# ansys/pychemkin

Hardware: AMD Instinct MI355X
Metric: reactor integrations/sec (GRI-3.0 const-P ignition) (higher is better)
Workload: dtype f64; 1 GPU; configs[2]: GRI-3.0 CONP CH4/air ignition sweep 64 T0 x 32 phi x 32 P per GPU; reactors_per_gpu=65536, ignition=TIFP, parallelism=shard-by-condition x1

## Files before the change

pychemkin_amd/csrc/ckmi_reactor.hpp:

```cpp
#pragma once
#include "ckmi_device.hpp"
#include "ckmi_image.hpp"
#include "../../include/ckmi.h"

namespace ckmi {

constexpr int QMAX = 5;
constexpr double ETAMX1 = 10000.0, ETAMX2 = 10.0, ETAMX3 = 10.0, ETAMXF = 0.2, ETAMIN = 0.1, ETACF = 0.25;
constexpr double ADDON = 1e-6, BIAS1 = 6.0, BIAS2 = 6.0, BIAS3 = 10.0, ONEPSM = 1.000001;
constexpr int SMALL_NST = 10, MXNCF = 10, MXNEF = 7, MXNEF1 = 3, SMALL_NEF = 2, LONG_WAIT = 10, MAXCOR = 3;
constexpr double CRDOWN = 0.3, DGMAX = 0.3, RDIV = 2.0, THRESH = 1.5, CORTES = 0.1;
constexpr int MSBP = 20, MSBJ = 15;
constexpr double UROUND = 2.220446049250313e-16, NNEG_TOL = 0.01;

constexpr int VL = WAVE;
struct WaveLds {
  int base;
  __device__ __forceinline__ double* C() const { return lds_at<double>(base); }
  __device__ __forceinline__ double* gRT() const { return lds_at<double>(base + 8 * VL); }
  __device__ __forceinline__ double* hRT() const { return lds_at<double>(base + 16 * VL); }
  __device__ __forceinline__ double* wdot() const { return lds_at<double>(base + 24 * VL); }
  __device__ __forceinline__ double* dwdT() const { return lds_at<double>(base + 32 * VL); }
  __device__ __forceinline__ double* ek() const { return lds_at<double>(base + 40 * VL); }
  __device__ __forceinline__ double* Mg() const { return lds_at<double>(base + 48 * VL); }
// ... 713 lines not shown
    if (wave_lane() >= n) b = 0.0;
    const double bp = bpermute(permv, b);
    double s0 = 0.0, s1 = 0.0;
#pragma unroll
    for (int j = 0; j < N; j += 2) {
      s0 = fma((double)a[j], bcast(bp, j), s0);
      if (j + 1 < N) s1 = fma((double)a[j + 1], bcast(bp, j + 1), s1);
    }
    return bpermute(permv, s0 + s1);
  }
};

template <int S>
__device__ __forceinline__ double pick(const double (&v)[S], int i) {
  double r = v[0];
#pragma unroll
  for (int k = 1; k < S; ++k) r = (i == k) ? v[k] : r;
  return r;
}

__device__ __forceinline__ double eta_root(double x, int p) {
  return (double)exp2f(log2f((float)x) / (float)p);
}

struct BdfS {
  double h, hscale, hprime, eta, etamax, hmax_inv, hmin, tn, rl1, gamma, gammap, gamrat, crate, acnrm, saved_tq5, hu;
  double l[QMAX + 1], tq[6], tau[QMAX + 2];
  int q, qprime, qwait, L, nst, nstlp, nstlj, jcur, ncf_tot, nef_tot, nlu, nfe, nje, nni;
  double rtol, atol;
  int nneg;
};

template <int ST>
struct ZnLdsT {
  int base;
  __device__ __forceinline__ double& operator[](int j) const { return *lds_at<double>(base + j * ST * 8); }
};
using ZnLds = ZnLdsT<WAVE>;
constexpr int ZN_BYTES = (QMAX + 1) * WAVE * 8;

template <int ST>
struct BdfT {
  ZnLdsT<ST> zn;
  double ewt, acor, tempv, ftemp, y;
};
using Bdf = BdfT<WAVE>;

__device__ __forceinline__ double wrms_lane(double v, double ewt, int n) {
  const double x = v * ewt;
  return sqrt(wave_sum(x * x) / n);
}

template <class BB, class SS>
__device__ __forceinline__ void bdf_rescale(BB& b, SS& S) {
  double factor = S.eta;
#pragma unroll
  for (int j = 1; j <= QMAX; ++j) {
    if (j <= S.q) {
      b.zn[j] *= factor;
      factor *= S.eta;
    }
  }
  S.h = S.hscale * S.eta;
  S.hscale = S.h;
}

template <class BB, class SS>
__device__ __forceinline__ void bdf_predict(BB& b, SS& S) {
  S.tn += S.h;
  const int q = S.q;
  double z[QMAX + 1];
#pragma unroll
  for (int j = 0; j <= QMAX; ++j) z[j] = b.zn[j];
#pragma unroll
  for (int k = 1; k <= QMAX; ++k)
#pragma unroll
    for (int j = QMAX; j >= 1; --j)
      if (j >= k) z[j - 1] = (k <= q && j <= q) ? z[j - 1] + z[j] : z[j - 1];
#pragma unroll
  for (int j = 0; j < QMAX; ++j) b.zn[j] = z[j];
}

template <class BB, class SS>
__device__ __forceinline__ void bdf_restore(BB& b, SS& S, double saved_t) {
  S.tn = saved_t;
  const int q = S.q;
  double z[QMAX + 1];
#pragma unroll
  for (int j = 0; j <= QMAX; ++j) z[j] = b.zn[j];
#pragma unroll
  for (int k = 1; k <= QMAX; ++k)
#pragma unroll
    for (int j = QMAX; j >= 1; --j)
      if (j >= k) z[j - 1] = (k <= q && j <= q) ? z[j - 1] - z[j] : z[j - 1];
#pragma unroll
  for (int j = 0; j < QMAX; ++j) b.zn[j] = z[j];
}

template <class BB, class SS>
__device__ __forceinline__ void bdf_set(BB& b, SS& S) {
  const int q = S.q;
  const double h = S.h;
  double tau[QMAX + 1];
#pragma unroll
  for (int i = 0; i <= QMAX; ++i) tau[i] = S.tau[i];
  double l[QMAX + 1];
  double xi_inv = 1.0, xistar_inv = 1.0, alpha0 = -1.0, alpha0_hat = -1.0, hsum = h;
  l[0] = l[1] = 1.0;
#pragma unroll
  for (int i = 2; i <= QMAX; ++i) l[i] = 0.0;
  if (q > 1) {
#pragma unroll
    for (int j = 2; j < QMAX; ++j) {
      if (j < q) {
        hsum += tau[j - 1];
        xi_inv = h / hsum;
// ... 6 lines not shown
    alpha0 -= 1.0 / q;
    xistar_inv = -l[1] - alpha0;
    double tq1 = tau[0];
#pragma unroll
    for (int i = 1; i <= QMAX; ++i) tq1 = (i == q - 1) ? tau[i] : tq1;
    hsum += tq1;
    xi_inv = h / hsum;
    alpha0_hat = -l[1] - xi_inv;
#pragma unroll
    for (int i = QMAX; i >= 1; --i)
      if (i <= q) l[i] += l[i - 1] * xistar_inv;
  }
  double lq = l[0];
#pragma unroll
  for (int i = 1; i <= QMAX; ++i) lq = (i == q) ? l[i] : lq;
#pragma unroll
  for (int i = 0; i <= QMAX; ++i) S.l[i] = l[i];
  const double A1 = 1.0 - alpha0_hat + alpha0;
  const double A2 = 1.0 + q * A1;
  const double tq2 = fabs(A1 / (alpha0 * A2));
  S.tq[2] = tq2;
  S.tq[5] = fabs(A2 * xistar_inv / (lq * xi_inv));
  if (S.qwait == 1) {
    if (q > 1) {
      const double Cc = xistar_inv / lq;
      const double A3 = alpha0 + 1.0 / q;
      const double A4 = alpha0_hat + xi_inv;
      const double Cpinv = (1.0 - A4 + A3) / A3;
      S.tq[1] = fabs(Cc * Cpinv);
    } else {
      S.tq[1] = 1.0;
    }
    double tq = tau[0];
#pragma unroll
    for (int i = 1; i <= QMAX; ++i) tq = (i == q) ? tau[i] : tq;
    hsum += tq;
    xi_inv = h / hsum;
    const double A5 = alpha0 - 1.0 / (q + 1);
    const double A6 = alpha0_hat - xi_inv;
    const double Cppinv = (1.0 - A6 + A5) / A2;
    S.tq[3] = fabs(Cppinv / (xi_inv * (q + 2) * A5));
  }
  S.tq[4] = CORTES / tq2;
  const double rl1 = 1.0 / l[1];
  const double gamma = h * rl1;
  S.rl1 = rl1;
  S.gamma = gamma;
  if (S.nst == 0) S.gammap = gamma;
  S.gamrat = (S.nst > 0) ? gamma / S.gammap : 1.0;
}


template <class BB, class SS>
__device__ __forceinline__ void bdf_adjust_order(BB& b, SS& S, int deltaq) {
  const int q = S.q;
#pragma unroll
  for (int i = 0; i <= QMAX; ++i) S.l[i] = 0.0;
  S.l[2] = 1.0;
  if (deltaq == 1) {
    double alpha1 = 1.0, prod = 1.0, xiold = 1.0, alpha0 = -1.0, hsum = S.hscale;
#pragma unroll
    for (int j = 1; j < QMAX; ++j) {
      if (j < q) {
        hsum += S.tau[j + 1];
        const double xi = hsum / S.hscale;
        prod *= xi;
        alpha0 -= 1.0 / (j + 1);
        alpha1 += 1.0 / xi;
#pragma unroll
        for (int i = QMAX; i >= 2; --i)
          if (i <= j + 2) S.l[i] = S.l[i] * xiold + S.l[i - 1];
        xiold = xi;
      }
    }
    const double A1 = (-alpha0 - alpha1) / prod;
    const double znL = A1 * b.zn[QMAX];
#pragma unroll
    for (int j = 2; j <= QMAX; ++j)
      if (j <= q) b.zn[j] += S.l[j] * znL;
#pragma unroll
    for (int j = 1; j <= QMAX; ++j)
      if (j == q + 1) b.zn[j] = znL;
  } else {
    double hsum = 0.0;
#pragma unroll
    for (int j = 1; j <= QMAX; ++j) {
      if (j <= q - 2) {
        hsum += S.tau[j];
        const double xi = hsum / S.hscale;
#pragma unroll
        for (int i = QMAX; i >= 2; --i)
          if (i <= j + 2) S.l[i] = S.l[i] * xi + S.l[i - 1];
      }
    }
    double znq = 0.0;
#pragma unroll
    for (int j = 0; j <= QMAX; ++j)
      if (j == q) znq = b.zn[j];
#pragma unroll
    for (int j = 2; j <= QMAX; ++j)
      if (j < q) b.zn[j] -= S.l[j] * znq;
  }
}

template <class BB, class SS>
__device__ __forceinline__ double dky0_lane(const BB& b, const SS& S, double t) {
  const double sc = (t - S.tn) / S.h;
  double v = 0.0;
#pragma unroll
  for (int j = QMAX; j >= 0; --j)
    if (j <= S.q) v = b.zn[j] + sc * v;
  return v;
}

}
```

pychemkin_amd/csrc/ckmi_reactor_kernel.hpp:

```cpp
#pragma once
#include <hip/hip_runtime.h>

#include <algorithm>
#include <string>
#include <type_traits>

#include "../../include/ckmi.h"
#include "ckmi_reactor.hpp"
#include "ckmi_run.hpp"
#include "ckmi_internal.hpp"

namespace {
using namespace ckmi;

enum { PH_RHS = 0, PH_JAC = 1, PH_LU = 2, PH_SOLVE = 3, PH_TOTAL = 4, PH_STATE = 8, PH_N = 48 };
#ifdef CKMI_PHASE_TIMERS
__device__ unsigned long long* g_phase_buf = nullptr;
#define PH_T0() const unsigned long long _ph0 = __builtin_amdgcn_s_memtime()
#define PH_ADD(slot) ph[slot] += __builtin_amdgcn_s_memtime() - _ph0
#else
#define PH_T0() (void)0
#define PH_ADD(slot) (void)0
#endif

// ... 55 lines not shown
  const ckmi_reactor_cfg* __restrict__ cfg = &dcfg->c;
  const int oJ = img.bytes;
  const int olock = oJ + jlock_offset(N);
  if (threadIdx.x == 0) *lds_at<int>(olock) = 0;
  stage_image(0, img);
  const MechView V = make_view(0, img);
  const int wid = threadIdx.x / WAVE;
  const int lane = threadIdx.x % WAVE;
  const int ows = oJ + jscratch_bytes<N>() + wid * (slice_bytes(img.G) + (PSR ? 8 * VL : 0));
  WaveLds L;
  L.base = ows;
  double* const Yin = PSR ? lds_at<double>(ows + slice_bytes(img.G)) : nullptr;
  const int oS = ows + slice_vec_bytes(img.G);
  BdfS& S = *lds_at<BdfS>(oS);
  Ctl& c = *lds_at<Ctl>(oS + align16((int)sizeof(BdfS)));
  Ign& g = *lds_at<Ign>(oS + align16((int)sizeof(BdfS)) + align16((int)sizeof(Ctl)));
  constexpr int RWAVES = rwaves(F64);
  float* Jg = reinterpret_cast<float*>(jws) + ((size_t)blockIdx.x * RWAVES + wid) * N * WAVE;
  const int KK = V.KK;
  const int n = KK + 1;
  const bool isp = lane >= 1 && lane <= KK;
  const bool act = lane < n;
  RunCtx& R = *lds_at<RunCtx>(oS + align16((int)sizeof(BdfS)) + align16((int)sizeof(Ctl)) + align16((int)sizeof(Ign)));
  R.cfg = cfg;
  std::conditional_t<F64, NewtonMatrixGJ64<N>, NewtonMatrixF32S<N>> M;
  Bdf b;
  b.zn.base = oS + align16((int)sizeof(BdfS)) + align16((int)sizeof(Ctl)) + align16((int)sizeof(Ign)) +
              align16((int)sizeof(RunCtx)) + lane * 8;
  double fe = 0.0, y_e = 0.0, t_e = 0.0;
  bool with_j = false;
#ifdef CKMI_PHASE_TIMERS
  unsigned long long ph[8] = {0, 0, 0, 0, 0, 0, 0, 0};
  unsigned long long t_r0 = 0;
  unsigned long long* phs = lds_at<unsigned long long>(oS + align16((int)sizeof(BdfS)) + align16((int)sizeof(Ctl)) +
                                                     align16((int)sizeof(Ign)) + align16((int)sizeof(RunCtx)) +
                                                     ZN_BYTES);
#endif
  int st = ST_NEXT;

#define REQUEST_F(T_, Y_, NEXT_) \
  do {                           \
    t_e = (T_);                  \
    y_e = (Y_);                  \
    with_j = false;              \
    st = (NEXT_);                \
    want = true;                 \
  } while (0)
#define START_BEGIN(T_, Y_, TOUT_, H0_)                                 \
  do {                                                                 \
    S.tn = (T_);                                                       \
    b.zn[0] = act ? (Y_) : 0.0;                                        \
    _Pragma("unroll") for (int j_ = 1; j_ <= QMAX; ++j_) b.zn[j_] = 0.0; \
    b.ewt = act ? 1.0 / (S.rtol * fabs(b.zn[0]) + S.atol) : 0.0;       \
    c.st_tout = (TOUT_);                                               \
    R.tsel = 0.5 * (S.tn + c.st_tout);                                 \
    c.st_h0 = (H0_);                                                   \
    REQUEST_F(S.tn, b.zn[0], ST_START_F);                              \
  } while (0)

  auto psr_resid = [&](double f, double y) -> double {
    if constexpr (PSR) {
      const double T = bcast(y, 0);
      const double sYW = wave_sum(isp ? y * V.rwt()[lane - 1] : 0.0);
      const double tau = R.pfr == 4 ? R.P0 / (RU * T * sYW * R.G) : 1.0 / R.G;
      const double den = lane == 0 ? io.ss_rtol * T : io.ss_rtol * fabs(y) + io.ss_atol;
      const double v = act ? tau * fabs(f) / den : 0.0;
      return __ballot(act && !(v == v)) != 0 ? __builtin_nan("") : wave_max(v);
    } else {
      return 0.0;
    }
  };

  for (;;) {
    bool want = false;
    while (!want && st != ST_EXIT) {
#ifdef CKMI_PHASE_TIMERS
      const int st_in = st;
      const unsigned long long t_st = __builtin_amdgcn_s_memtime();
#endif
      if constexpr (PSR) {
        if (st == ST_FINISH && c.stopped == 0) {
          c.stopped = 2;
          REQUEST_F(S.tn, b.zn[0], ST_PSR_END_F);
          continue;
        }
        if (st > ST_EXIT) {
          S.nfe++;
          const double res = psr_resid(fe, y_e);
          if (st == ST_PSR_END_F) {
            c.avar_last = res;
            if (c.status == 0 && !(res <= 1.0)) c.status = CKMI_RUN_NOT_STEADY;
            st = ST_FINISH;
            continue;
          }
          const bool polishing = st == ST_PSR_POLISH_F;
          if (res <= 1.0) {
            if (polishing) b.zn[0] = b.y;
            c.avar_last = res;
            c.stopped = 1;
            st = ST_FINISH;
            continue;
          }
          if (polishing ? (c.nadap < PSR_POLISH_ITERS && res < PSR_POLISH_RATE * c.delp) : res <= PSR_POLISH_MAX) {
            c.nadap = polishing ? c.nadap + 1 : 1;
            c.delp = res;
            const double d = M.solve(act ? S.gammap * fe : 0.0, n);
            S.nni++;
// ... 62 lines not shown
          R.mass = R.rho0 * R.V0;
          if (PF && R.pfr == 1) {
            R.G = R.rho0 * R.V0;
            R.Pm = R.P0 + R.G * R.V0;
          }
          if constexpr (PSR) {
            const bool vgiven = io.mode == 2;
            R.conp = 1;
            R.pfr = vgiven ? 4 : 3;
            const double Tin = io.Tin[r], mdot = io.mdot[r];
            const double yi = isp ? io.Yin[(size_t)r * KK + lane - 1] : 0.0;
            if (isp) Yin[lane - 1] = yi;
            const double hin = isp ? nasa7_img(V, lane - 1, Tin, log(Tin), 1.0 / Tin).hRT * RU * Tin * V.rwt()[lane - 1] : 0.0;
            R.Pm = wave_sum(yi * hin);
            R.G = vgiven ? mdot / R.V0 : 1.0 / R.V0;
            R.mass = vgiven ? R.rho0 * R.V0 : R.V0 * mdot;
            wave_lds_sync();
          }
          R.gfac = cfg->gfac;
          R.qloss = cfg->qloss;
          R.htc = cfg->htc;
          R.areaq = cfg->areaq;
          R.tamb = cfg->tamb;
          R.nq = cfg->prof2_kind == 1 ? cfg->nprof2 : 0;
          R.na = cfg->prof2_kind == 2 ? cfg->nprof2 : cfg->nprof3;
          R.a_t = cfg->prof2_kind == 2 ? cfg->prof2_t : cfg->prof3_t;
          R.a_v = cfg->prof2_kind == 2 ? cfg->prof2_v : cfg->prof3_v;
          {
            const int ar = io.afac_rxn ? io.afac_rxn[r] : -1;
            R.pslot = (ar >= 0 && ar < img.II) ? img.slot_of[ar] : -1;
            R.plnf = R.pslot >= 0 ? log(io.afac[r]) : 0.0;
          }
          c.nadap = 0;
          c.avar_last = bcast(yl, cfg->avar > 0 ? cfg->avar : 0);
          c.T0 = T0;
          c.yguard = dcfg->guard_y;
          c.tguard_lo = dcfg->guard_tlo;
          c.tguard_hi = dcfg->guard_thi;
          S.rtol = cfg->rtol;
          S.atol = cfg->atol;
          S.nneg = cfg->nneg;
          S.ncf_tot = S.nef_tot = S.nlu = S.nfe = S.nje = S.nni = 0;
          c.tend = cfg->t_end;
          if constexpr (PSR) {
            if (!(c.tend > 0.0)) c.tend = 1000.0 * (R.pfr == 4 ? R.rho0 / R.G : 1.0 / R.G);
          }
          c.hmax = cfg->hmax > 0.0 ? cfg->hmax : c.tend / 100.0;
          S.hmax_inv = 1.0 / c.hmax;
          S.hmin = 0.0;
          c.ncrit = n_crit(dcfg);
          c.icrit = 0;
          c.first = 1;
          c.max_steps = cfg->max_steps > 0 ? cfg->max_steps : 200000;
#ifdef CKMI_PHASE_TIMERS
#pragma unroll
          for (int k = 0; k < 8; ++k) ph[k] = 0;
          if (lane < 40) phs[lane] = 0;
          t_r0 = __builtin_amdgcn_s_memtime();
#endif
          START_BEGIN(0.0, yl, crit_time(dcfg, c.tend, 0), cfg->h0);
          break;
        }
        case ST_START_F: {
          b.zn[1] = act ? fe : 0.0;
          S.nfe++;
          if (c.st_h0 > 0.0) {
            c.st_h = c.st_h0;
            st = ST_START_FINISH;
            break;
          }
          const double t0 = S.tn, tout = c.st_tout;
          const double tdist = fabs(tout - t0);
          const double tround = UROUND * fmax(fabs(t0), fabs(tout));
          const double hlb = 100.0 * tround;
          double hub = 0.1 * tdist;
          const double num = act ? fabs(b.zn[1]) : 0.0;
          const double den = 0.1 * fabs(b.zn[0]) + S.atol;
          const double hub_inv = wave_max(act ? num / (den > 0 ? den : 1e-300) : 0.0);
          if (hub * hub_inv > 1.0) hub = 1.0 / hub_inv;
          const double hg = sqrt(hlb * hub);
          if (hub < hlb) {
            c.st_h = hg;
            st = ST_START_FINISH;
            break;
          }
          c.is_t0 = t0;
          c.is_hg = hg;
          c.is_hub = hub;
          c.is_hlb = hlb;
          c.is_count = 1;
          REQUEST_F(t0 + hg, b.zn[0] + hg * b.zn[1], ST_INITSTEP_F);
          break;
        }
        case ST_INITSTEP_F: {
          S.nfe++;
          const double hg = c.is_hg, hub = c.is_hub;
          const double f1 = act ? (fe - b.zn[1]) / hg : 0.0;
          const double yddnrm = wrms_lane(f1, b.ewt, n);
          double hnew = (yddnrm * hub * hub > 2.0) ? sqrt(2.0 / yddnrm) : sqrt(hg * hub);
          bool done = c.is_count == 4;
          if (!done) {
            const double hrat = hnew / hg;
            if (hrat > 0.5 && hrat < 2.0) {
              done = true;
            } else if (c.is_count >= 2 && hrat > 2.0) {
              hnew = hg;
// ... 17 lines not shown
          double h = c.st_h;
          if (h > c.hmax) h = c.hmax;
          if (h > c.st_tout - S.tn) h = c.st_tout - S.tn;
          b.zn[1] *= h;
          S.h = S.hscale = S.hprime = h;
          S.q = S.qprime = 1;
          S.L = 2;
          S.qwait = S.L;
          S.etamax = ETAMX1;
          S.nst = 0;
          S.nstlp = 0;
          S.nstlj = 0;
          S.jcur = 0;
          S.crate = 1.0;
          S.gammap = S.gamma = S.h;
          S.gamrat = 1.0;
          S.saved_tq5 = 0.0;
#pragma unroll
          for (int i = 0; i <= QMAX + 1; ++i) S.tau[i] = 0.0;
#pragma unroll
          for (int i = 0; i < 6; ++i) S.tq[i] = 0.0;
          S.hu = 0.0;
          st = ST_STEP_BEGIN;
          if (c.first) {
            c.first = 0;
            g.mode = cfg->ign_mode;
            g.comp = (g.mode == 4) ? 1 + cfg->ign_species : 0;
            g.found = g.started = g.have_prev = g.have_next = 0;
            g.thresh = 0.0;
            g.best = -1e300;
            g.tbest = g.tprev = g.vprev = g.tnext = g.vnext = g.tlast = g.vlast = 0.0;
            g.tau = -1.0;
            if (g.mode == 2) g.thresh = c.T0 + cfg->ign_val;
            if (g.mode == 3) g.thresh = cfg->ign_val;
            c.isave = 0;
            while (c.isave < io.nsave && io.t_save[c.isave] <= 0.0) {
              if (act) io.y_save[((size_t)c.r * io.nsave + c.isave) * n + lane] = b.zn[0];
              c.isave++;
            }
            c.status = 0;
            c.nst = 0;
            c.stopped = 0;
            if (g.mode == 1 || g.mode == 4) REQUEST_F(0.0, b.zn[0], ST_IGN0_F);
          }
          break;
        }
        case ST_IGN0_F: {
          S.nfe++;
          ign_peak_update(g, 0.0, g.mode == 1 ? bcast(fe, 0) : bcast(b.zn[0], g.comp));
          st = ST_STEP_BEGIN;
          break;
        }
        case ST_STEP_BEGIN: {
          if (!(S.tn < c.tend * (1.0 - 1e-15))) {
            st = ST_FINISH;
            break;
          }

          c.tc = crit_time(dcfg, c.tend, c.icrit);
          if (S.tn + S.hprime > c.tc) {
            const double hp = c.tc - S.tn;
            S.eta = hp / S.h;
            if (S.nst > 0) {
              S.hprime = hp;
            } else {
              bdf_rescale(b, S);
              S.hprime = S.h;
            }
          }
          b.ewt = act ? 1.0 / (S.rtol * fabs(b.zn[0]) + S.atol) : 0.0;
          c.told = S.tn;
          c.saved_t = S.tn;
          c.ncf = c.nef = 0;
          c.nflag = NF_FIRST;
          if (S.nst > 0 && S.hprime != S.h) {
            if (S.qprime != S.q) {
              bdf_adjust_order(b, S, S.qprime - S.q);
              S.q = S.qprime;
              S.L = S.q + 1;
              S.qwait = S.L;
            }
            bdf_rescale(b, S);
          }
          st = ST_STEP_ATTEMPT;
          break;
        }
        case ST_STEP_ATTEMPT: {
          bdf_predict(b, S);
          bdf_set(b, S);
          c.convfail = (c.nflag == NF_FIRST || c.nflag == NF_ERR_FAIL) ? CF_NONE : CF_OTHER;
          c.call_setup = (c.nflag != NF_FIRST) || S.nst == 0 || S.nst >= S.nstlp + MSBP || fabs(S.gamrat - 1.0) > DGMAX;
          st = ST_NLS_ATTEMPT;
          break;
        }
        case ST_NLS_ATTEMPT: {
          b.y = b.zn[0];
          if (c.call_setup) {
            const double dgamma = fabs(S.gamma / S.gammap - 1.0);
            const int jbad = S.nst == 0 || S.nst >= S.nstlj + MSBJ || (c.convfail == CF_BAD_J && dgamma < DGMAX) ||
                             c.convfail == CF_OTHER;
            if (jbad) {
              REQUEST_F(S.tn, b.y, ST_NLS_J);
              with_j = true;
              break;
            }
          }
          REQUEST_F(S.tn, b.y, ST_NLS_F);
          break;
        }
        case ST_NLS_F: {
          b.ftemp = fe;
          S.nfe++;
          if (!c.call_setup) {
            b.acor = 0.0;
            c.delp = 0.0;
            c.mm = 0;
            st = ST_NEWTON_ITER;
            break;
          }
          S.jcur = 0;
          st = ST_SETUP;
          break;
        }
        case ST_NLS_J: {
          b.ftemp = fe;
          {
            const double* Jsh = lds_at<const double>(oJ);
#pragma unroll 2
            for (int j = 0; j < N; ++j) Jg[j * WAVE + lane] = (float)Jsh[j * LDJ + lane];
          }
          wave_lds_sync();
          if (lane == 0) atomicExch(lds_at<int>(olock), 0);
          S.nfe += 2;
          S.nje++;
          S.nstlj = S.nst;
          S.jcur = 1;
          st = ST_SETUP;
          break;
        }
        case ST_SETUP: {
#ifdef CKMI_PHASE_TIMERS
          const unsigned long long t0 = __builtin_amdgcn_s_memtime();
#endif
          const bool ok = M.build_factor(Jg, WAVE, S.gamma, n, L.base + 32 * VL);
#ifdef CKMI_PHASE_TIMERS
          ph[PH_LU] += __builtin_amdgcn_s_memtime() - t0;
#endif
          S.nlu++;
          S.crate = 1.0;
          S.gammap = S.gamma;
          S.gamrat = 1.0;
          S.nstlp = S.nst;
          if (!ok) {
            st = ST_STEP_CONVFAIL;
            break;
          }
          b.acor = 0.0;
          c.delp = 0.0;
          c.mm = 0;
          st = ST_NEWTON_ITER;
          break;
        }
        case ST_NEWTON_ITER: {
          const double rhs = act ? S.gamma * b.ftemp - (S.rl1 * b.zn[1] + b.acor) : 0.0;
#ifdef CKMI_PHASE_TIMERS
          const unsigned long long t0 = __builtin_amdgcn_s_memtime();
#endif
          double x = M.solve(rhs, n);
#ifdef CKMI_PHASE_TIMERS
          ph[PH_SOLVE] += __builtin_amdgcn_s_memtime() - t0;
#endif
          S.nni++;
          if (S.gamrat != 1.0) x *= 2.0 / (1.0 + S.gamrat);
          if (!act) x = 0.0;
          const double z0 = b.zn[0];
          b.acor += x;
          b.y = z0 + b.acor;
          const bool neg = S.nneg && act && lane >= 1 && b.y < 0.0;
          double nv[4];
          {
            const double xe = x * b.ewt, ae = b.acor * b.ewt, ne = neg ? b.y * b.ewt : 0.0;
            const double fe2 = neg ? z0 * b.ewt : ae;
            nv[0] = xe * xe;
            nv[1] = ae * ae;
            nv[2] = ne * ne;
            nv[3] = fe2 * fe2;
          }
          wave_sum_multi<4>(nv, lane);
          const double del = sqrt(nv[0] / n);
          if (c.mm > 0) S.crate = fmax(CRDOWN * S.crate, del / c.delp);
          const double dcon = del * fmin(1.0, S.crate) / S.tq[4];
          if (dcon <= 1.0) {
            bool negfail = false, negfix = false;
            if (S.nneg && nv[2] > 0.0) {
              if (sqrt(nv[2] / n) > NNEG_TOL) {
                negfail = true;
              } else {
                negfix = true;
                if (neg) {
                  b.y = 0.0;
                  b.acor = -z0;
                }
              }
            }
            if (negfail) {
              c.failed = 2;
              st = ST_NLS_FAIL;
              break;
            }
            S.acnrm = (c.mm == 0 && !negfix) ? del : sqrt((negfix ? nv[3] : nv[1]) / n);
            S.jcur = 0;
            st = ST_ERRTEST;
            break;
          }
          c.mm++;
          if (c.mm == MAXCOR || (c.mm >= 2 && del > RDIV * c.delp)) {
            c.failed = 1;
            st = ST_NLS_FAIL;
            break;
          }
          c.delp = del;
          REQUEST_F(S.tn, b.y, ST_NEWTON_F);
          break;
        }
        case ST_NEWTON_F: {
          b.ftemp = fe;
          S.nfe++;
          st = ST_NEWTON_ITER;
          break;
        }
        case ST_NLS_FAIL: {
          if (c.failed == 1 && !S.jcur) {
            c.convfail = CF_BAD_J;
            c.call_setup = 1;
            st = ST_NLS_ATTEMPT;
          } else {
            st = ST_STEP_CONVFAIL;
          }
          break;
        }
        case ST_STEP_CONVFAIL: {
          c.ncf++;
          S.ncf_tot++;
          S.etamax = 1.0;
          bdf_restore(b, S, c.saved_t);
          if (fabs(S.h) <= S.hmin * ONEPSM || c.ncf == MXNCF) {
            c.rc = CKMI_RUN_CONVFAIL;
            st = ST_STEP_END;
            break;
          }
          S.eta = fmax(ETACF, S.hmin / fabs(S.h));
          c.nflag = NF_CONV_FAIL;
          bdf_rescale(b, S);
          st = ST_STEP_ATTEMPT;
          break;
        }
        case ST_ERRTEST: {
          c.dsm = S.acnrm * S.tq[2];
          if (c.dsm <= 1.0) {
            st = ST_STEP_COMPLETE;
            break;
          }
          c.nef++;
          S.nef_tot++;
          c.nflag = NF_ERR_FAIL;
          bdf_restore(b, S, c.saved_t);
          if (fabs(S.h) <= S.hmin * ONEPSM || c.nef == MXNEF) {
            c.rc = CKMI_RUN_ERRTEST;
            st = ST_STEP_END;
            break;
          }
          S.etamax = 1.0;
          st = ST_STEP_ATTEMPT;
          if (c.nef <= MXNEF1) {
            S.eta = 1.0 / (eta_root(BIAS2 * c.dsm, S.L) + ADDON);
            S.eta = fmax(ETAMIN, fmax(S.eta, S.hmin / fabs(S.h)));
            if (c.nef >= SMALL_NEF) S.eta = fmin(S.eta, ETAMXF);
            bdf_rescale(b, S);
            break;
          }
          if (S.q > 1) {
            S.eta = fmax(ETAMIN, S.hmin / fabs(S.h));
            bdf_adjust_order(b, S, -1);
            S.L = S.q;
            S.q--;
            S.qwait = S.L;
            bdf_rescale(b, S);
            break;
          }
          S.eta = fmax(ETAMIN, S.hmin / fabs(S.h));
          S.h *= S.eta;
          S.hscale = S.h;
          S.qwait = LONG_WAIT;
          REQUEST_F(S.tn, b.zn[0], ST_ERR_F);
          break;
        }
        case ST_ERR_F: {
          S.nfe++;
          b.zn[1] = act ? S.h * fe : 0.0;
          st = ST_STEP_ATTEMPT;
          break;
        }
        case ST_STEP_COMPLETE: {
          const double dsm = c.dsm;
          S.nst++;
          c.nst++;
          S.hu = S.h;
#pragma unroll
          for (int i = QMAX; i >= 2; --i)
            if (i <= S.q) S.tau[i] = S.tau[i - 1];
          if (S.q == 1 && S.nst > 1) S.tau[2] = S.tau[1];
          S.tau[1] = S.h;
          double ddn = 0.0, dup = 0.0;
          if (S.etamax != 1.0 && S.qwait == 1) {
            const bool qm = S.q > 1, qp = S.q != QMAX && S.saved_tq5 != 0.0;
            double cquot = 0.0;
            if (qp) {
              const double hr = S.h / S.tau[2];
              double hrL = hr;
              for (int j = 1; j < S.L; ++j) hrL *= hr;
              cquot = (S.tq[5] / S.saved_tq5) * hrL;
            }
            double ov[2];
            {
              double znq = 0.0, lq = 0.0;
#pragma unroll
              for (int j = 0; j <= QMAX; ++j)
                if (j == S.q) {
                  znq = b.zn[j];
                  lq = S.l[j];
                }
              const double a = (act && qm) ? (znq + lq * b.acor) * b.ewt : 0.0;
              const double t = (act && qp) ? (b.acor - cquot * b.zn[QMAX]) * b.ewt : 0.0;
              ov[0] = a * a;
              ov[1] = t * t;
            }
            wave_sum_multi<2>(ov, lane);
            ddn = sqrt(ov[0] / n) * S.tq[1];
            dup = sqrt(ov[1] / n) * S.tq[3];
          }
          if (dcfg->npe) elem_project_wave(V, dcfg->npe, c.eb0, S.rtol, b.zn[0], b.acor, lane, L.ek());
#pragma unroll
          for (int j = 0; j <= QMAX; ++j)
            if (j <= S.q) b.zn[j] += S.l[j] * b.acor;
          S.qwait--;
          if (S.qwait == 1 && S.q != QMAX) {
            b.zn[QMAX] = b.acor;
            S.saved_tq5 = S.tq[5];
          }
          if (S.etamax == 1.0) {
            if (S.qwait < 2) S.qwait = 2;
            S.qprime = S.q;
            S.hprime = S.h;
            S.eta = 1.0;
          } else {
            const double etaq = 1.0 / (eta_root(BIAS2 * dsm, S.L) + ADDON);
            if (S.qwait != 0) {
              S.eta = etaq;
              S.qprime = S.q;
            } else {
              S.qwait = 2;
              double etaqm1 = 0.0, etaqp1 = 0.0;
              if (S.q > 1) etaqm1 = 1.0 / (eta_root(BIAS1 * ddn, S.q) + ADDON);
              if (S.q != QMAX && S.saved_tq5 != 0.0) etaqp1 = 1.0 / (eta_root(BIAS3 * dup, S.L + 1) + ADDON);
              const double etam = fmax(etaqm1, fmax(etaq, etaqp1));
              if (etam < THRESH) {
                S.eta = 1.0;
                S.qprime = S.q;
              } else if (etam == etaq) {
                S.eta = etaq;
                S.qprime = S.q;
              } else if (etam == etaqm1) {
                S.eta = etaqm1;
                S.qprime = S.q - 1;
              } else {
                S.eta = etaqp1;
                S.qprime = S.q + 1;
                b.zn[QMAX] = b.acor;
              }
            }
            if (S.eta < THRESH) {
              S.eta = 1.0;
              S.hprime = S.h;
            } else {
              S.eta = fmin(S.eta, S.etamax);
              S.eta /= fmax(1.0, fabs(S.h) * S.hmax_inv * S.eta);
              S.hprime = S.h * S.eta;
            }
          }
          S.etamax = (S.nst <= SMALL_NST) ? ETAMX2 : ETAMX3;
          {
            const double z0 = b.zn[0];
            const bool bad = isp ? -z0 > c.yguard
                                 : (lane == 0 && R.energy == 1 && !(z0 >= c.tguard_lo && z0 <= c.tguard_hi));
            c.rc = __ballot(bad) != 0 ? CKMI_RUN_RUNAWAY : 0;
          }
          if constexpr (PF) {
            if (R.pfr == 1 && R.npv == 0 && c.rc == 0) {
              const double z0 = b.zn[0];
              const double sYW = wave_sum(isp ? z0 * V.rwt()[lane - 1] : 0.0);
              if (R.Pm * R.Pm - 4.0 * R.G * R.G * RU * bcast(z0, 0) * sYW < 0.0) c.rc = CKMI_RUN_CHOKED;
            }
          }
          st = ST_STEP_END;
          break;
        }
        case ST_STEP_END: {
          if (c.rc != 0) {
            c.status = c.rc;
            st = ST_FINISH;
            break;
          }
          const double tn = S.tn;
          while (c.isave < io.nsave && io.t_save[c.isave] <= tn) {
            const double ys = dky0_lane(b, S, io.t_save[c.isave]);
            if (act) io.y_save[((size_t)c.r * io.nsave + c.isave) * n + lane] = ys;
            c.isave++;
          }
          if (g.mode == 1) {
            ign_peak_update(g, tn, bcast(b.zn[1], 0) / S.h);
          } else if (g.mode == 4) {
            ign_peak_update(g, tn, bcast(b.zn[0], g.comp));
          } else if ((g.mode == 2 || g.mode == 3) && !g.found && bcast(b.zn[0], 0) >= g.thresh) {
            double lo = c.told, hi = tn;
            for (int it = 0; it < 60; ++it) {
              const double mid = 0.5 * (lo + hi);
              if (bcast(dky0_lane(b, S, mid), 0) >= g.thresh) hi = mid;
              else lo = mid;
            }
            g.found = 1;
            g.tau = hi;
          }
          st = ST_STEP_BEGIN;
          if (cfg->ign_stop) {
            if ((g.mode == 2 || g.mode == 3) && g.found) {
              c.stopped = 1;
              st = ST_FINISH;
              break;
            }
            if (g.mode == 1 && g.have_next && g.vlast < 0.1 * g.best && bcast(b.zn[0], 0) > c.T0 + 200.0) {
              c.stopped = 1;
              st = ST_FINISH;
              break;
            }
          }
          bool adap = false;
          if (io.n_adap && c.nadap < io.max_adap) {
            if (cfg->asteps > 0 && c.nst % cfg->asteps == 0) adap = true;
            if (cfg->avar >= 0 && cfg->avalue > 0.0) {
              const double v = bcast(b.zn[0], cfg->avar);
              if (fabs(v - c.avar_last) >= cfg->avalue) adap = true;
            }
          }
          if (adap) {
            const size_t a = (size_t)c.r * io.max_adap + c.nadap;
            if (lane == 0) io.t_adap[a] = tn;
            if (act) io.y_adap[a * n + lane] = b.zn[0];
            c.nadap++;
            if (cfg->avar >= 0) c.avar_last = bcast(b.zn[0], cfg->avar);
          }
          if (c.nst >= c.max_steps) {
            c.status = CKMI_RUN_MAXSTEPS;
            st = ST_FINISH;
            break;
          }
          if (tn >= c.tc * (1.0 - 1e-15) && c.icrit < c.ncrit - 1) {
            c.icrit++;
            START_BEGIN(tn, b.zn[0], crit_time(dcfg, c.tend, c.icrit), 0.0);
          }
          if constexpr (PSR) {
            if (st == ST_STEP_BEGIN && psr_resid(b.zn[1] / S.h, b.zn[0]) <= PSR_SCREEN)
              REQUEST_F(tn, b.zn[0], ST_PSR_SS_F);
          }
          break;
        }
        case ST_FINISH: {
          double yf;
          double tf = c.tend;
          if (c.stopped || c.status) {
            tf = S.tn;
            yf = b.zn[0];
          } else {
            yf = dky0_lane(b, S, c.tend);
          }
          if (g.mode == 1 || g.mode == 4) g.tau = ign_peak_time(g);
          double Pf, Vf;
          state_PV<PF>(V, R, tf, yf, lane, Pf, Vf);
          const int r = c.r;
          while (c.isave < io.nsave) {
            if (act) io.y_save[((size_t)r * io.nsave + c.isave) * n + lane] = __builtin_nan("");
            c.isave++;
          }
          if (io.t_stop && lane == 0) io.t_stop[r] = tf;
          if constexpr (PSR) {
            const double sYW = wave_sum(isp ? yf * V.rwt()[lane - 1] : 0.0);
            const double rho = R.P0 / (RU * bcast(yf, 0) * sYW);
            if (lane == 0) {
              io.rho[r] = rho;
              io.tau_res[r] = R.pfr == 4 ? rho / R.G : 1.0 / R.G;
              io.vol[r] = R.pfr == 4 ? R.V0 : R.mass / rho;
              io.resid[r] = c.avar_last;
            }
          }
          if (lane == 0) {
            if constexpr (!PSR) io.tau[r] = g.tau;
            io.T[r] = yf;
            if constexpr (!PSR) {
              io.P[r] = Pf;
              io.V[r] = Vf;
            }
            int* sto = io.stats + (size_t)r * CKMI_NSTAT;
            sto[CKMI_STAT_NST] = c.nst;
            sto[CKMI_STAT_NFE] = S.nfe;
            sto[CKMI_STAT_NJE] = S.nje;
            sto[CKMI_STAT_NLU] = S.nlu;
            sto[CKMI_STAT_NCF] = S.ncf_tot;
            sto[CKMI_STAT_NEF] = S.nef_tot;
            sto[CKMI_STAT_STATUS] = c.status;
            sto[CKMI_STAT_NNI] = S.nni;
// ... 214 lines not shown
```

pychemkin_amd/csrc/ckmi_run.hpp:

```cpp
#pragma once
#include "ckmi_reactor.hpp"

namespace ckmi {

enum { NF_FIRST = 0, NF_CONV_FAIL = 1, NF_ERR_FAIL = 2 };
enum { CF_NONE = 0, CF_BAD_J = 1, CF_OTHER = 2 };

struct Ign {
  int mode, comp, found, started, have_prev, have_next;
  double thresh, best, tbest, tprev, vprev, tnext, vnext, tlast, vlast, tau;
};

__device__ __forceinline__ void ign_peak_update(Ign& g, double t, double v) {
  if (g.started && g.found == 0 && v > g.best) {
    g.tprev = g.tlast;
    g.vprev = g.vlast;
    g.have_prev = 1;
    g.best = v;
    g.tbest = t;
    g.have_next = 0;
  } else if (g.started && !g.have_next && g.tbest != 0.0 && t > g.tbest) {
    g.tnext = t;
    g.vnext = v;
    g.have_next = 1;
// ... 24 lines not shown
struct DevCfg {
  ckmi_reactor_cfg c;
  int ncrit;
  double tcrit[192];
  double guard_y, guard_tlo, guard_thi;
  int npe;
};
__device__ __forceinline__ bool runaway_value_bad(const DevCfg* d, double T) {
  return !(T >= d->guard_tlo && T <= d->guard_thi);
}
__device__ __forceinline__ int n_crit(const DevCfg* d) { return d->ncrit + 1; }
__device__ __forceinline__ double crit_time(const DevCfg* d, double tend, int idx) {
  return idx < d->ncrit ? d->tcrit[idx] : tend;
}

struct ReactorIO {
  const int* problem;
  const double *T0, *P0, *V0, *Y0;
  double *tau, *T, *P, *V, *Y;
  int* stats;
  int nsave;
  const double* t_save;
  double* y_save;
  const int* afac_rxn;
  const double* afac;
  int max_adap;
  double* t_adap;
  double* y_adap;
  int* n_adap;
  double* t_stop;
};

struct PsrIO : ReactorIO {
  const double *Tin, *Yin, *mdot, *tau_or_vol;
  double *rho, *tau_res, *vol, *resid;
  int mode;
  double ss_rtol, ss_atol;
};

struct ProbeIO {
  const int* problem;
  const double *T0, *P0, *V0, *Y0, *t, *y;
  const int* afac_rxn;
  const double* afac;
  const double *Tin, *Yin, *mdot;
  int mode;
  double *f, *J;
};
constexpr int PROBE_GRID_MAX = 64;

struct Ctl {
  int r, first, nflag, convfail, call_setup, failed, mm, ncf, nef, rc, isave, icrit, ncrit, status, nst, stopped;
  int is_count, max_steps, nadap;
  double avar_last;
  double delp, saved_t, told, dsm, tc, tend, hmax, T0;
  double yguard, tguard_lo, tguard_hi;
  double st_h0, st_tout, st_h, is_hg, is_hub, is_hlb, is_t0;
  double eb0[PROJ_MMAX];
  double tdh;
};

__host__ __device__ constexpr int align16(int b) { return (b + 15) & ~15; }

enum {
  ST_NEXT = 0,
  ST_START_F,
  ST_INITSTEP_F,
  ST_START_FINISH,
  ST_IGN0_F,
  ST_STEP_BEGIN,
  ST_STEP_ATTEMPT,
  ST_NLS_ATTEMPT,
  ST_NLS_F,
  ST_NLS_J,
  ST_SETUP,
  ST_NEWTON_ITER,
  ST_NEWTON_F,
  ST_NLS_FAIL,
  ST_STEP_CONVFAIL,
  ST_ERRTEST,
  ST_ERR_F,
  ST_STEP_COMPLETE,
  ST_STEP_END,
  ST_FINISH,
  ST_EXIT,
  ST_PSR_SS_F,
  ST_PSR_POLISH_F,
  ST_PSR_END_F
};

}
```

Before: 92780 reactors/s.

## Cache BDF state in registers and precompute per-reactor config flags in step loop

Rewrites the BDF history helpers (rescale, adjust_order, dky, correct history, tau shift) to load Nordsieck and tau arrays into local registers, update them with branch-free selects and write back once. Step-begin, Newton, and step-complete states read state fields into locals before use. A bitmask of config options (crit times, ign stop, save, adaptive output, element projection) is computed once per reactor so the step-end path skips global config loads. The critical-time lookup moves from every step to START_BEGIN, which adds coupling that must keep tc correct when the crit index advances.

```diff
diff --git a/pychemkin_amd/csrc/ckmi_reactor.hpp b/pychemkin_amd/csrc/ckmi_reactor.hpp
--- a/pychemkin_amd/csrc/ckmi_reactor.hpp
+++ b/pychemkin_amd/csrc/ckmi_reactor.hpp
@@ -789,16 +789,21 @@
 }
 
 template <class BB, class SS>
-__device__ __forceinline__ void bdf_rescale(BB& b, SS& S) {
-  double factor = S.eta;
+__host__ __device__ __forceinline__ void bdf_rescale(BB& b, SS& S) {
+  const int q = S.q;
+  const double eta = S.eta;
+  double z[QMAX + 1];
+#pragma unroll
+  for (int j = 1; j <= QMAX; ++j) z[j] = b.zn[j];
+  double factor = eta;
 #pragma unroll
   for (int j = 1; j <= QMAX; ++j) {
-    if (j <= S.q) {
-      b.zn[j] *= factor;
-      factor *= S.eta;
-    }
-  }
-  S.h = S.hscale * S.eta;
+    z[j] = (j <= q) ? z[j] * factor : z[j];
+    factor = (j <= q) ? factor * eta : factor;
+  }
+#pragma unroll
+  for (int j = 1; j <= QMAX; ++j) b.zn[j] = z[j];
+  S.h = S.hscale * eta;
   S.hscale = S.h;
 }
 
@@ -911,65 +916,107 @@
 
 
 template <class BB, class SS>
-__device__ __forceinline__ void bdf_adjust_order(BB& b, SS& S, int deltaq) {
+__host__ __device__ __forceinline__ void bdf_adjust_order(BB& b, SS& S, int deltaq) {
   const int q = S.q;
-#pragma unroll
-  for (int i = 0; i <= QMAX; ++i) S.l[i] = 0.0;
-  S.l[2] = 1.0;
+  const double hscale = S.hscale;
+  double tau[QMAX + 1];
+#pragma unroll
+  for (int i = 1; i <= QMAX; ++i) tau[i] = S.tau[i];
+  double z[QMAX + 1];
+#pragma unroll
+  for (int j = 0; j <= QMAX; ++j) z[j] = b.zn[j];
+  double l[QMAX + 1];
+#pragma unroll
+  for (int i = 0; i <= QMAX; ++i) l[i] = 0.0;
+  l[2] = 1.0;
   if (deltaq == 1) {
-    double alpha1 = 1.0, prod = 1.0, xiold = 1.0, alpha0 = -1.0, hsum = S.hscale;
+    double alpha1 = 1.0, prod = 1.0, xiold = 1.0, alpha0 = -1.0, hsum = hscale;
 #pragma unroll
     for (int j = 1; j < QMAX; ++j) {
       if (j < q) {
-        hsum += S.tau[j + 1];
-        const double xi = hsum / S.hscale;
+        hsum += tau[j + 1];
+        const double xi = hsum / hscale;
         prod *= xi;
         alpha0 -= 1.0 / (j + 1);
         alpha1 += 1.0 / xi;
 #pragma unroll
         for (int i = QMAX; i >= 2; --i)
-          if (i <= j + 2) S.l[i] = S.l[i] * xiold + S.l[i - 1];
+          if (i <= j + 2) l[i] = l[i] * xiold + l[i - 1];
         xiold = xi;
       }
     }
     const double A1 = (-alpha0 - alpha1) / prod;
-    const double znL = A1 * b.zn[QMAX];
-#pragma unroll
-    for (int j = 2; j <= QMAX; ++j)
-      if (j <= q) b.zn[j] += S.l[j] * znL;
-#pragma unroll
-    for (int j = 1; j <= QMAX; ++j)
-      if (j == q + 1) b.zn[j] = znL;
+    const double znL = A1 * z[QMAX];
+#pragma unroll
+    for (int j = 2; j <= QMAX; ++j) z[j] = (j <= q) ? z[j] + l[j] * znL : z[j];
+#pragma unroll
+    for (int j = 1; j <= QMAX; ++j) z[j] = (j == q + 1) ? znL : z[j];
   } else {
     double hsum = 0.0;
 #pragma unroll
     for (int j = 1; j <= QMAX; ++j) {
       if (j <= q - 2) {
-        hsum += S.tau[j];
-        const double xi = hsum / S.hscale;
+        hsum += tau[j];
+        const double xi = hsum / hscale;
 #pragma unroll
         for (int i = QMAX; i >= 2; --i)
-          if (i <= j + 2) S.l[i] = S.l[i] * xi + S.l[i - 1];
+          if (i <= j + 2) l[i] = l[i] * xi + l[i - 1];
       }
     }
     double znq = 0.0;
 #pragma unroll
-    for (int j = 0; j <= QMAX; ++j)
-      if (j == q) znq = b.zn[j];
-#pragma unroll
-    for (int j = 2; j <= QMAX; ++j)
-      if (j < q) b.zn[j] -= S.l[j] * znq;
-  }
+    for (int j = 0; j <= QMAX; ++j) znq = (j == q) ? z[j] : znq;
+#pragma unroll
+    for (int j = 2; j <= QMAX; ++j) z[j] = (j < q) ? z[j] - l[j] * znq : z[j];
+  }
+#pragma unroll
+  for (int i = 0; i <= QMAX; ++i) S.l[i] = l[i];
+#pragma unroll
+  for (int j = 1; j <= QMAX; ++j) b.zn[j] = z[j];
 }
 
 template <class BB, class SS>
-__device__ __forceinline__ double dky0_lane(const BB& b, const SS& S, double t) {
+__host__ __device__ __forceinline__ double dky0_lane(const BB& b, const SS& S, double t) {
+  const int q = S.q;
   const double sc = (t - S.tn) / S.h;
+  double z[QMAX + 1];
+#pragma unroll
+  for (int j = 0; j <= QMAX; ++j) z[j] = b.zn[j];
   double v = 0.0;
 #pragma unroll
-  for (int j = QMAX; j >= 0; --j)
-    if (j <= S.q) v = b.zn[j] + sc * v;
+  for (int j = QMAX; j >= 0; --j) v = (j <= q) ? z[j] + sc * v : v;
   return v;
 }
 
-}
+template <class BB, class SS>
+__host__ __device__ __forceinline__ void bdf_correct_history(BB& b, const SS& S, int q, bool park) {
+  const double acor = b.acor;
+  double z[QMAX + 1], l[QMAX + 1];
+#pragma unroll
+  for (int j = 0; j <= QMAX; ++j) {
+    z[j] = b.zn[j];
+    l[j] = S.l[j];
+  }
+#pragma unroll
+  for (int j = 0; j <= QMAX; ++j) z[j] = (j <= q) ? z[j] + l[j] * acor : z[j];
+  z[QMAX] = park ? acor : z[QMAX];
+#pragma unroll
+  for (int j = 0; j <= QMAX; ++j) b.zn[j] = z[j];
+}
+
+template <class SS>
+__host__ __device__ __forceinline__ double bdf_tau_shift(SS& S, int q, int nst, double h) {
+  double t[QMAX + 1];
+#pragma unroll
+  for (int i = 1; i <= QMAX; ++i) t[i] = S.tau[i];
+  double u[QMAX + 1];
+#pragma unroll
+  for (int i = QMAX; i >= 2; --i) u[i] = (i <= q) ? t[i - 1] : t[i];
+  u[2] = (q == 1 && nst > 1) ? t[1] : u[2];
+  u[1] = h;
+#pragma unroll
+  for (int i = 1; i <= QMAX; ++i) S.tau[i] = u[i];
+  return u[2];
+}
+
+}
diff --git a/pychemkin_amd/csrc/ckmi_reactor_kernel.hpp b/pychemkin_amd/csrc/ckmi_reactor_kernel.hpp
--- a/pychemkin_amd/csrc/ckmi_reactor_kernel.hpp
+++ b/pychemkin_amd/csrc/ckmi_reactor_kernel.hpp
@@ -131,7 +131,7 @@
     b.zn[0] = act ? (Y_) : 0.0;                                        \
     _Pragma("unroll") for (int j_ = 1; j_ <= QMAX; ++j_) b.zn[j_] = 0.0; \
     b.ewt = act ? 1.0 / (S.rtol * fabs(b.zn[0]) + S.atol) : 0.0;       \
-    c.st_tout = (TOUT_);                                               \
+    c.tc = c.st_tout = (TOUT_);       \
     R.tsel = 0.5 * (S.tn + c.st_tout);                                 \
     c.st_h0 = (H0_);                                                   \
     REQUEST_F(S.tn, b.zn[0], ST_START_F);                              \
@@ -300,6 +300,9 @@
           c.icrit = 0;
           c.first = 1;
           c.max_steps = cfg->max_steps > 0 ? cfg->max_steps : 200000;
+          c.flags = (dcfg->ncrit > 0 ? SF_CRIT : 0) | (cfg->ign_stop ? SF_IGN_STOP : 0) | (io.nsave > 0 ? SF_SAVE : 0) |
+                    (io.n_adap ? SF_ADAP : 0) | (cfg->asteps > 0 ? SF_ASTEPS : 0) | (cfg->avar >= 0 ? SF_AVAR : 0) |
+                    (dcfg->npe << SF_NPE_SHIFT);
 #ifdef CKMI_PHASE_TIMERS
 #pragma unroll
           for (int k = 0; k < 8; ++k) ph[k] = 0;
@@ -423,33 +426,35 @@
           break;
         }
         case ST_STEP_BEGIN: {
-          if (!(S.tn < c.tend * (1.0 - 1e-15))) {
+          const double tn = S.tn, tend = c.tend, tc = c.tc, h = S.h, rtol = S.rtol, atol = S.atol, z0 = b.zn[0];
+          double hprime = S.hprime;
+          const int nst = S.nst, q = S.q, qprime = S.qprime;
+          if (!(tn < tend * (1.0 - 1e-15))) {
             st = ST_FINISH;
             break;
           }
-
-          c.tc = crit_time(dcfg, c.tend, c.icrit);
-          if (S.tn + S.hprime > c.tc) {
-            const double hp = c.tc - S.tn;
-            S.eta = hp / S.h;
-            if (S.nst > 0) {
+          if (tn + hprime > tc) {
+            const double hp = tc - tn;
+            S.eta = hp / h;
+            if (nst > 0) {
+              hprime = hp;
               S.hprime = hp;
             } else {
               bdf_rescale(b, S);
               S.hprime = S.h;
             }
           }
-          b.ewt = act ? 1.0 / (S.rtol * fabs(b.zn[0]) + S.atol) : 0.0;
-          c.told = S.tn;
-          c.saved_t = S.tn;
+          b.ewt = act ? 1.0 / (rtol * fabs(z0) + atol) : 0.0;
+          c.told = tn;
+          c.saved_t = tn;
           c.ncf = c.nef = 0;
           c.nflag = NF_FIRST;
-          if (S.nst > 0 && S.hprime != S.h) {
-            if (S.qprime != S.q) {
-              bdf_adjust_order(b, S, S.qprime - S.q);
-              S.q = S.qprime;
-              S.L = S.q + 1;
-              S.qwait = S.L;
+          if (nst > 0 && hprime != h) {
+            if (qprime != q) {
+              bdf_adjust_order(b, S, qprime - q);
+              S.q = qprime;
+              S.L = qprime + 1;
+              S.qwait = qprime + 1;
             }
             bdf_rescale(b, S);
           }
@@ -459,17 +464,22 @@
         case ST_STEP_ATTEMPT: {
           bdf_predict(b, S);
           bdf_set(b, S);
-          c.convfail = (c.nflag == NF_FIRST || c.nflag == NF_ERR_FAIL) ? CF_NONE : CF_OTHER;
-          c.call_setup = (c.nflag != NF_FIRST) || S.nst == 0 || S.nst >= S.nstlp + MSBP || fabs(S.gamrat - 1.0) > DGMAX;
+          {
+            const int nflag = c.nflag, nst = S.nst, nstlp = S.nstlp;
+            const double gamrat = S.gamrat;
+            c.convfail = (nflag == NF_FIRST || nflag == NF_ERR_FAIL) ? CF_NONE : CF_OTHER;
+            c.call_setup = (nflag != NF_FIRST) | (nst == 0) | (nst >= nstlp + MSBP) | (fabs(gamrat - 1.0) > DGMAX);
+          }
           st = ST_NLS_ATTEMPT;
           break;
         }
         case ST_NLS_ATTEMPT: {
           b.y = b.zn[0];
           if (c.call_setup) {
+            const int nst = S.nst, nstlj = S.nstlj, convfail = c.convfail;
             const double dgamma = fabs(S.gamma / S.gammap - 1.0);
-            const int jbad = S.nst == 0 || S.nst >= S.nstlj + MSBJ || (c.convfail == CF_BAD_J && dgamma < DGMAX) ||
-                             c.convfail == CF_OTHER;
+            const int jbad = (nst == 0) | (nst >= nstlj + MSBJ) | ((convfail == CF_BAD_J) & (dgamma < DGMAX)) |
+                             (convfail == CF_OTHER);
             if (jbad) {
               REQUEST_F(S.tn, b.y, ST_NLS_J);
               with_j = true;
@@ -541,13 +551,14 @@
 #ifdef CKMI_PHASE_TIMERS
           ph[PH_SOLVE] += __builtin_amdgcn_s_memtime() - t0;
 #endif
+          const double gamrat = S.gamrat, crate0 = S.crate, tq4 = S.tq[4], delp = c.delp, z0 = b.zn[0];
+          const int nneg = S.nneg, mm = c.mm;
           S.nni++;
-          if (S.gamrat != 1.0) x *= 2.0 / (1.0 + S.gamrat);
+          if (gamrat != 1.0) x *= 2.0 / (1.0 + gamrat);
           if (!act) x = 0.0;
-          const double z0 = b.zn[0];
           b.acor += x;
           b.y = z0 + b.acor;
-          const bool neg = S.nneg && act && lane >= 1 && b.y < 0.0;
+          const bool neg = nneg && act && lane >= 1 && b.y < 0.0;
           double nv[4];
           {
             const double xe = x * b.ewt, ae = b.acor * b.ewt, ne = neg ? b.y * b.ewt : 0.0;
@@ -559,11 +570,15 @@
           }
           wave_sum_multi<4>(nv, lane);
           const double del = sqrt(nv[0] / n);
-          if (c.mm > 0) S.crate = fmax(CRDOWN * S.crate, del / c.delp);
-          const double dcon = del * fmin(1.0, S.crate) / S.tq[4];
+          double crate = crate0;
+          if (mm > 0) {
+            crate = fmax(CRDOWN * crate0, del / delp);
+            S.crate = crate;
+          }
+          const double dcon = del * fmin(1.0, crate) / tq4;
           if (dcon <= 1.0) {
             bool negfail = false, negfix = false;
-            if (S.nneg && nv[2] > 0.0) {
+            if (nneg && nv[2] > 0.0) {
               if (sqrt(nv[2] / n) > NNEG_TOL) {
                 negfail = true;
               } else {
@@ -579,13 +594,13 @@
               st = ST_NLS_FAIL;
               break;
             }
-            S.acnrm = (c.mm == 0 && !negfix) ? del : sqrt((negfix ? nv[3] : nv[1]) / n);
+            S.acnrm = (mm == 0 && !negfix) ? del : sqrt((negfix ? nv[3] : nv[1]) / n);
             S.jcur = 0;
             st = ST_ERRTEST;
             break;
           }
-          c.mm++;
-          if (c.mm == MAXCOR || (c.mm >= 2 && del > RDIV * c.delp)) {
+          c.mm = mm + 1;
+          if (mm + 1 == MAXCOR || (mm + 1 >= 2 && del > RDIV * delp)) {
             c.failed = 1;
             st = ST_NLS_FAIL;
             break;
@@ -673,93 +688,93 @@
           break;
         }
         case ST_STEP_COMPLETE: {
-          const double dsm = c.dsm;
-          S.nst++;
+          const double dsm = c.dsm, h = S.h, etamax = S.etamax, hmax_inv = S.hmax_inv, tq5 = S.tq[5];
+          double saved_tq5 = S.saved_tq5;
+          const int q = S.q, Lq = S.L, nst = S.nst + 1, fl = c.flags;
+          int qwait = S.qwait;
+          S.nst = nst;
           c.nst++;
-          S.hu = S.h;
-#pragma unroll
-          for (int i = QMAX; i >= 2; --i)
-            if (i <= S.q) S.tau[i] = S.tau[i - 1];
-          if (S.q == 1 && S.nst > 1) S.tau[2] = S.tau[1];
-          S.tau[1] = S.h;
+          S.hu = h;
+          const double tau2 = bdf_tau_shift(S, q, nst, h);
           double ddn = 0.0, dup = 0.0;
-          if (S.etamax != 1.0 && S.qwait == 1) {
-            const bool qm = S.q > 1, qp = S.q != QMAX && S.saved_tq5 != 0.0;
+          if (etamax != 1.0 && qwait == 1) {
+            const bool qm = q > 1, qp = q != QMAX && saved_tq5 != 0.0;
+            const double tq1 = S.tq[1], tq3 = S.tq[3];
             double cquot = 0.0;
             if (qp) {
-              const double hr = S.h / S.tau[2];
+              const double hr = h / tau2;
               double hrL = hr;
-              for (int j = 1; j < S.L; ++j) hrL *= hr;
-              cquot = (S.tq[5] / S.saved_tq5) * hrL;
+              for (int j = 1; j < Lq; ++j) hrL *= hr;
+              cquot = (tq5 / saved_tq5) * hrL;
             }
             double ov[2];
             {
-              double znq = 0.0, lq = 0.0;
+              double znq = 0.0, lq = 0.0, znQ = 0.0;
 #pragma unroll
-              for (int j = 0; j <= QMAX; ++j)
-                if (j == S.q) {
-                  znq = b.zn[j];
-                  lq = S.l[j];
-                }
+              for (int j = 0; j <= QMAX; ++j) {
+                const double zj = b.zn[j], lj = S.l[j];
+                znq = (j == q) ? zj : znq;
+                lq = (j == q) ? lj : lq;
+                if (j == QMAX) znQ = zj;
+              }
               const double a = (act && qm) ? (znq + lq * b.acor) * b.ewt : 0.0;
-              const double t = (act && qp) ? (b.acor - cquot * b.zn[QMAX]) * b.ewt : 0.0;
+              const double t = (act && qp) ? (b.acor - cquot * znQ) * b.ewt : 0.0;
               ov[0] = a * a;
               ov[1] = t * t;
             }
             wave_sum_multi<2>(ov, lane);
-            ddn = sqrt(ov[0] / n) * S.tq[1];
-            dup = sqrt(ov[1] / n) * S.tq[3];
-          }
-          if (dcfg->npe) elem_project_wave(V, dcfg->npe, c.eb0, S.rtol, b.zn[0], b.acor, lane, L.ek());
-#pragma unroll
-          for (int j = 0; j <= QMAX; ++j)
-            if (j <= S.q) b.zn[j] += S.l[j] * b.acor;
-          S.qwait--;
-          if (S.qwait == 1 && S.q != QMAX) {
-            b.zn[QMAX] = b.acor;
-            S.saved_tq5 = S.tq[5];
-          }
-          if (S.etamax == 1.0) {
-            if (S.qwait < 2) S.qwait = 2;
-            S.qprime = S.q;
-            S.hprime = S.h;
-            S.eta = 1.0;
+            ddn = sqrt(ov[0] / n) * tq1;
+            dup = sqrt(ov[1] / n) * tq3;
+          }
+          if (const int npe = fl >> SF_NPE_SHIFT) elem_project_wave(V, npe, c.eb0, S.rtol, b.zn[0], b.acor, lane, L.ek());
+          qwait--;
+          const bool park = qwait == 1 && q != QMAX;
+          bdf_correct_history(b, S, q, park);
+          if (park) saved_tq5 = tq5;
+          double eta, hprime;
+          int qprime = q;
+          if (etamax == 1.0) {
+            if (qwait < 2) qwait = 2;
+            hprime = h;
+            eta = 1.0;
           } else {
-            const double etaq = 1.0 / (eta_root(BIAS2 * dsm, S.L) + ADDON);
-            if (S.qwait != 0) {
-              S.eta = etaq;
-              S.qprime = S.q;
+            const double etaq = 1.0 / (eta_root(BIAS2 * dsm, Lq) + ADDON);
+            if (qwait != 0) {
+              eta = etaq;
             } else {
-              S.qwait = 2;
+              qwait = 2;
               double etaqm1 = 0.0, etaqp1 = 0.0;
-              if (S.q > 1) etaqm1 = 1.0 / (eta_root(BIAS1 * ddn, S.q) + ADDON);
-              if (S.q != QMAX && S.saved_tq5 != 0.0) etaqp1 = 1.0 / (eta_root(BIAS3 * dup, S.L + 1) + ADDON);
+              if (q > 1) etaqm1 = 1.0 / (eta_root(BIAS1 * ddn, q) + ADDON);
+              if (q != QMAX && saved_tq5 != 0.0) etaqp1 = 1.0 / (eta_root(BIAS3 * dup, Lq + 1) + ADDON);
               const double etam = fmax(etaqm1, fmax(etaq, etaqp1));
               if (etam < THRESH) {
-                S.eta = 1.0;
-                S.qprime = S.q;
+                eta = 1.0;
               } else if (etam == etaq) {
-                S.eta = etaq;
-                S.qprime = S.q;
+                eta = etaq;
               } else if (etam == etaqm1) {
-                S.eta = etaqm1;
-                S.qprime = S.q - 1;
+                eta = etaqm1;
+                qprime = q - 1;
               } else {
-                S.eta = etaqp1;
-                S.qprime = S.q + 1;
+                eta = etaqp1;
+                qprime = q + 1;
                 b.zn[QMAX] = b.acor;
               }
             }
-            if (S.eta < THRESH) {
-              S.eta = 1.0;
-              S.hprime = S.h;
+            if (eta < THRESH) {
+              eta = 1.0;
+              hprime = h;
             } else {
-              S.eta = fmin(S.eta, S.etamax);
-              S.eta /= fmax(1.0, fabs(S.h) * S.hmax_inv * S.eta);
-              S.hprime = S.h * S.eta;
-            }
-          }
-          S.etamax = (S.nst <= SMALL_NST) ? ETAMX2 : ETAMX3;
+              eta = fmin(eta, etamax);
+              eta /= fmax(1.0, fabs(h) * hmax_inv * eta);
+              hprime = h * eta;
+            }
+          }
+          S.qwait = qwait;
+          S.saved_tq5 = saved_tq5;
+          S.qprime = qprime;
+          S.hprime = hprime;
+          S.eta = eta;
+          S.etamax = (nst <= SMALL_NST) ? ETAMX2 : ETAMX3;
           {
             const double z0 = b.zn[0];
             const bool bad = isp ? -z0 > c.yguard
@@ -777,22 +792,25 @@
           break;
         }
         case ST_STEP_END: {
-          if (c.rc != 0) {
-            c.status = c.rc;
+          const int rc = c.rc, fl = c.flags, gmode = g.mode, nst = c.nst, max_steps = c.max_steps;
+          const double tn = S.tn;
+          if (rc != 0) {
+            c.status = rc;
             st = ST_FINISH;
             break;
           }
-          const double tn = S.tn;
-          while (c.isave < io.nsave && io.t_save[c.isave] <= tn) {
-            const double ys = dky0_lane(b, S, io.t_save[c.isave]);
-            if (act) io.y_save[((size_t)c.r * io.nsave + c.isave) * n + lane] = ys;
-            c.isave++;
-          }
-          if (g.mode == 1) {
+          if (fl & SF_SAVE) {
+            while (c.isave < io.nsave && io.t_save[c.isave] <= tn) {
+              const double ys = dky0_lane(b, S, io.t_save[c.isave]);
+              if (act) io.y_save[((size_t)c.r * io.nsave + c.isave) * n + lane] = ys;
+              c.isave++;
+            }
+          }
+          if (gmode == 1) {
             ign_peak_update(g, tn, bcast(b.zn[1], 0) / S.h);
-          } else if (g.mode == 4) {
+          } else if (gmode == 4) {
             ign_peak_update(g, tn, bcast(b.zn[0], g.comp));
-          } else if ((g.mode == 2 || g.mode == 3) && !g.found && bcast(b.zn[0], 0) >= g.thresh) {
+          } else if ((gmode == 2 || gmode == 3) && !g.found && bcast(b.zn[0], 0) >= g.thresh) {
             double lo = c.told, hi = tn;
             for (int it = 0; it < 60; ++it) {
               const double mid = 0.5 * (lo + hi);
@@ -803,22 +821,22 @@
             g.tau = hi;
           }
           st = ST_STEP_BEGIN;
-          if (cfg->ign_stop) {
-            if ((g.mode == 2 || g.mode == 3) && g.found) {
+          if (fl & SF_IGN_STOP) {
+            if ((gmode == 2 || gmode == 3) && g.found) {
               c.stopped = 1;
               st = ST_FINISH;
               break;
             }
-            if (g.mode == 1 && g.have_next && g.vlast < 0.1 * g.best && bcast(b.zn[0], 0) > c.T0 + 200.0) {
+            if (gmode == 1 && g.have_next && g.vlast < 0.1 * g.best && bcast(b.zn[0], 0) > c.T0 + 200.0) {
               c.stopped = 1;
               st = ST_FINISH;
               break;
             }
           }
           bool adap = false;
-          if (io.n_adap && c.nadap < io.max_adap) {
-            if (cfg->asteps > 0 && c.nst % cfg->asteps == 0) adap = true;
-            if (cfg->avar >= 0 && cfg->avalue > 0.0) {
+          if ((fl & SF_ADAP) && c.nadap < io.max_adap) {
+            if ((fl & SF_ASTEPS) && nst % cfg->asteps == 0) adap = true;
+            if ((fl & SF_AVAR) && cfg->avalue > 0.0) {
               const double v = bcast(b.zn[0], cfg->avar);
               if (fabs(v - c.avar_last) >= cfg->avalue) adap = true;
             }
@@ -828,14 +846,14 @@
             if (lane == 0) io.t_adap[a] = tn;
             if (act) io.y_adap[a * n + lane] = b.zn[0];
             c.nadap++;
-            if (cfg->avar >= 0) c.avar_last = bcast(b.zn[0], cfg->avar);
-          }
-          if (c.nst >= c.max_steps) {
+            if (fl & SF_AVAR) c.avar_last = bcast(b.zn[0], cfg->avar);
+          }
+          if (nst >= max_steps) {
             c.status = CKMI_RUN_MAXSTEPS;
             st = ST_FINISH;
             break;
           }
-          if (tn >= c.tc * (1.0 - 1e-15) && c.icrit < c.ncrit - 1) {
+          if ((fl & SF_CRIT) && tn >= c.tc * (1.0 - 1e-15) && c.icrit < c.ncrit - 1) {
             c.icrit++;
             START_BEGIN(tn, b.zn[0], crit_time(dcfg, c.tend, c.icrit), 0.0);
           }
diff --git a/pychemkin_amd/csrc/ckmi_run.hpp b/pychemkin_amd/csrc/ckmi_run.hpp
--- a/pychemkin_amd/csrc/ckmi_run.hpp
+++ b/pychemkin_amd/csrc/ckmi_run.hpp
@@ -100,12 +100,24 @@
 struct Ctl {
   int r, first, nflag, convfail, call_setup, failed, mm, ncf, nef, rc, isave, icrit, ncrit, status, nst, stopped;
   int is_count, max_steps, nadap;
+  int flags;
   double avar_last;
   double delp, saved_t, told, dsm, tc, tend, hmax, T0;
   double yguard, tguard_lo, tguard_hi;
   double st_h0, st_tout, st_h, is_hg, is_hub, is_hlb, is_t0;
   double eb0[PROJ_MMAX];
   double tdh;
+};
+
+static_assert(offsetof(Ctl, avar_last) == 80, "Ctl::flags takes the padding behind the ints: the slice keeps its size");
+enum {
+  SF_CRIT = 1,
+  SF_IGN_STOP = 2,
+  SF_SAVE = 4,
+  SF_ADAP = 8,
+  SF_ASTEPS = 16,
+  SF_AVAR = 32,
+  SF_NPE_SHIFT = 8
 };
 
 __host__ __device__ constexpr int align16(int b) { return (b + 15) & ~15; }
```

Result: faster. 93810 reactors/s (median of 6 runs) (+1.1%).
